# ImpulseAdventure/JPEGsnoop

Measured on AMD Instinct MI355X. Metric: Mpixels/sec decoded (baseline 4:2:0 JPEG) at 1/2/4/8 GPUs; bit-exact vs ref, higher is better.
Workload: dtype u8/i16 entropy+DIB, f32 IDCT+colour; 1 GPU; 1024 x 1920x1080 baseline 4:2:0 q85 JPEG per GPU (64 distinct seeds replicated; BASELINE config 3, config 4 at 8 GPUs), HBM->HBM (T1); images_per_gpu=1024, distinct=64, subsampling=4:2:0, quality=85, parallelism=single, decode_form=two halves on two streams (library default)

## Files before the change

jpegsnoop_amd/csrc/jsnoop_host.cpp:

```cpp
#include <hip/hip_runtime.h>
#include <math.h>
#include <stdarg.h>
#include <stdio.h>
#include <stdlib.h>
#include <string.h>
#include <string>
#include <vector>
#include <chrono>
#include <algorithm>
#include <atomic>
#include "../../include/jsnoop_gpu.h"
#include "jsnoop_types.h"
#include "jsnoop_launch.h"
#include "jsnoop_host.h"
#include "jsnoop_bytes.h"

static thread_local std::string g_err;
void js_set_error(const char* fmt, ...)
{
    char buf[1024]; va_list ap; va_start(ap, fmt); vsnprintf(buf, sizeof buf, fmt, ap); va_end(ap); g_err = buf;
}
#define HIP_TRY(expr) do { hipError_t e_ = (expr); if (e_ != hipSuccess) { \
    js_set_error("%s failed: %s (%s:%d)", #expr, hipGetErrorString(e_), __FILE__, __LINE__); return -1; } } while (0)

// ... 411 lines not shown
        syb[n + 1 + i] = snw; snw += (im.n_subseq + JS_SY_THREADS - JS_SY_HALO - 1) / (JS_SY_THREADS - JS_SY_HALO);
        max_mcu_h = std::max(max_mcu_h, im.mcu_h); max_mcu_w = std::max(max_mcu_w, im.mcu_w);
        wg[i] = wgs; wgs += std::max(1u, (nmcu + 8 * mcus_per_wave - 1) / (8 * mcus_per_wave));
    }
    usb[n] = usc; usb[2 * n + 1] = us4; syb[n] = syw; syb[2 * n + 1] = snw; us_chunks = usc; sy_wgs = syw; sn_wgs = snw; seg_words = segw; mcu_bytes = mcub;
    wg[n] = wgs; total_wgs = wgs; rec_words = recw; total_blocks = blocks; dib_bytes = dibb; side_words = side; total_subseq = subs; ustr_bytes = ustr;
    if (grow(&dev.raw, &cap.raw, raw_bytes + 64) || grow(&dev.coef, &cap.coef, blocks * 128) || grow(&dev.dccum, &cap.dccum, blocks * 2 + 64) ||
        grow(&dev.dib, &cap.dib, dibb) || grow(&dev.side, &cap.side, side * 4) || grow(&dev.imgs, &cap.imgs, n * sizeof(JsImage)) ||
        grow(&dev.tables, &cap.tables, tables.size() * sizeof(JsTableSet)) || grow(&dev.wg_base, &cap.wg_base, (n + 1) * 4) ||
        grow(&dev.sel, &cap.sel, n * 4) || grow(&dev.sums, &cap.sums, n * 8) || grow(&dev.ustr, &cap.ustr, ustr + 64) ||
        grow(&dev.sub, &cap.sub, subs * 24 + 64 + js_sync_list_words(subs, (uint32_t)n) * 4) || grow(&dev.probe, &cap.probe, 1024) || grow(&dev.seg, &cap.seg, segw * 4 + 64) ||
        grow(&dev.chunk_keep, &cap.chunk_keep, (size_t)usc * 4 + 64) || grow(&dev.chunk_rst, &cap.chunk_rst, (size_t)usc * 4 + 64) ||
        grow(&dev.us_base, &cap.us_base, 2 * (n + 1) * 4) || grow(&dev.sy_base, &cap.sy_base, 2 * (n + 1) * 4) ||
        grow(&dev.mcu_rst, &cap.mcu_rst, mcub + 64) || grow(&dev.dc_parts, &cap.dc_parts, JS_DC_PARTS_BYTES) || grow(&dev.ustr_lin, &cap.ustr_lin, ustr + 64) || grow(&dev.flags, &cap.flags, n * 8 + 64) ||
        grow(&dev.us_state, &cap.us_state, (size_t)usc * 8 + 64)) return -1;
    HIP_TRY(hipMemsetAsync(dev.us_state, 0, (size_t)usc * 8 + 64, stream)); us_epoch = 0; us_ticket_base[0] = us_ticket_base[1] = 0;
    if (opt_want_planes && grow(&dev.planes, &cap.planes, plane * 2)) return -1;
    { uint32_t most = 0; for (size_t i = 0; i < n; i++) most = std::max(most, wg[i + 1] - wg[i]); if (most > 64 && grow(&dev.wg_part, &cap.wg_part, (size_t)wgs * 16 + 64)) return -1; }
    cand_blk = max_blk; cand_rounds = (cand_fits && sub_wl == 4) ? cand_want : -1;
    cand_half = cand_rounds >= 0 && tune.write_lanes != 1 && (subs <= 40960 || tune.write_lanes == 2);
    if (cand_rounds >= 0 && (grow(&dev.cand, &cap.cand, js_cand_bytes(subs)) || grow(&dev.cand_req, &cap.cand_req, n * JS_CAND_REQ_WORDS * 4))) return -1;
    event_words = opt_events ? (uint64_t)n * (1 + JS_EV_WORDS * JS_EV_MAX) : 0;
    if (event_words && grow(&dev.events, &cap.events, event_words * 4)) return -1;
    tab_rows = 1; tab_lut2 = 0; uint32_t tdc = 1, tac = 1;
    for (const JsTableSet& t : tables) { tab_rows = std::max(tab_rows, t.n_rows); tab_lut2 = std::max(tab_lut2, t.lut2_used); tdc = std::max(tdc, t.n_dc_rows); tac = std::max(tac, t.n_ac_rows); }
    tab_rows_w = tdc | (tac << 8);
    HIP_TRY(hipMemcpyAsync(dev.raw, pinned, raw_bytes, hipMemcpyHostToDevice, stream));
    {
        const size_t sz[5] = { n * sizeof(JsImage), tables.size() * sizeof(JsTableSet), (n + 1) * 4, 2 * (n + 1) * 4, 2 * (n + 1) * 4 };
        const void* src[5] = { imgs.data(), tables.data(), wg.data(), usb.data(), syb.data() };
        void* dst[5] = { dev.imgs, dev.tables, dev.wg_base, dev.us_base, dev.sy_base };
// ... 73 lines not shown
{
    HIP_TRY(hipSetDevice(device));
    if (!uploaded && upload()) return -1;
    const uint32_t n = (uint32_t)imgs.size();
    last_form = (!force_generic && dc_fast_applies()) ? 2 : 1;
    side_done.assign(n, 0); side_mode.assign(n, 0); side_anoms.assign(n, std::vector<uint32_t>()); side_chunk_ok.assign(n, 0); side_events.assign(n, std::vector<uint32_t>()); side_pre.assign(n, 0); side_requests = 0;
    JsRange r_("jsnoop:decode (enqueue)");
    if (js_prog_count(this)) return decode_progressive(timed);
    if (timed) HIP_TRY(hipEventRecord(ev[0], stream));
    us_epoch = us_epoch % 255u + 1u;
    bool parallel_ok = !opt_force_exact; if (parallel_ok) { parallel_ok = false; for (const JsTableSet& t : tables) parallel_ok = parallel_ok || t.lut_ok; }
    if (!parallel_ok) {
        HIP_TRY(hipMemsetAsync(dev.coef, 0, total_blocks * 128, stream));
        HIP_TRY(hipMemsetAsync(dev.dccum, 0, total_blocks * 2, stream));
    }
    js_launch_clear3(stream, dev.side, side_words * 4, dev.mcu_rst, mcu_bytes, dev.flags, (size_t)n * 8, parallel_ok ? dev.imgs : nullptr, n);
    if (event_words) HIP_TRY(hipMemsetAsync(dev.events, 0, event_words * 4, stream));
    if (timed) HIP_TRY(hipEventRecord(ev[1], stream));
    last_timed_split = false;
    if (split_parts == 2 && parallel_ok && !event_words) {
        if (ensure_aux()) return -1;
        const uint32_t n0 = n / 2; hipStream_t s2 = aux[0];
        HIP_TRY(hipEventRecord(aux_ev[0], stream)); HIP_TRY(hipStreamWaitEvent(s2, aux_ev[0], 0));
        if (js_parallel_entropy_part(this, stream, 0, n0, timed ? ev : nullptr, aux_ev[2], 1) < 0) return -1;
        HIP_TRY(hipStreamWaitEvent(s2, aux_ev[2], 0));
        if (timed) { HIP_TRY(hipEventRecord(ev2[0], s2)); HIP_TRY(hipEventRecord(ev2[1], s2)); }
        if (js_parallel_entropy_part(this, s2, n0, n - n0, timed ? ev2 : nullptr) < 0) return -1;
        last_used_parallel = true;
        if (timed) { HIP_TRY(hipEventRecord(ev[7], stream)); HIP_TRY(hipEventRecord(ev2[7], s2)); }
        { JsRange r2_("jsnoop:idct+colour"); if (launch_back_end_part(stream, 0, n0) || launch_back_end_part(s2, n0, n - n0)) return -1; }
        if (timed) { HIP_TRY(hipEventRecord(ev[8], stream)); HIP_TRY(hipEventRecord(ev2[8], s2)); last_timed_split = true; }
// ... 764 lines not shown
```

jpegsnoop_amd/csrc/jsnoop_host.h:

```cpp
#pragma once
#include <hip/hip_runtime.h>
#include <stdint.h>
#include <string>
#include <utility>
#include <vector>
#include "../../include/jsnoop_gpu.h"
#include "jsnoop_types.h"

struct JsTables {
    uint16_t dqt_nat[4][64], dqt_zz[4][64]; int dqt_sel[256];
    int      dht_sel[2][5];
    uint32_t dht_setmax[2], dht_size[2][4];
    uint32_t dht_bitlen[2][4][JS_DHT_CODES], dht_bits[2][4][JS_DHT_CODES], dht_mask[2][4][JS_DHT_CODES], dht_code[2][4][JS_DHT_CODES];
    uint32_t dht_fast[2][4][2 << JS_FAST_BITS];
    uint32_t dht_histo_unused[1];
    int      details_set; uint32_t dim_x, dim_y, num_sof, num_sos, precision;
    uint32_t samp_h[256], samp_v[256];
    int      rst_en; uint32_t rst_interval;
};

struct JsnoopBatch;
struct JsProgBatch;

struct JsnoopDecoder {
// ... 68 lines not shown
    bool last_timed_split = false;
    bool last_used_parallel = false;
    int  last_form = 0;
    bool force_generic = false;
    bool private_no_log = false;
    bool dc_fast_applies() const;
    int  redecode_generic();
    int  ensure_generic();
    uint32_t* d_side_tmp = nullptr; size_t side_tmp_cap = 0;
    uint8_t* pinned; size_t pinned_cap; uint64_t raw_bytes;
    uint8_t* d2h_land = nullptr;
    uint8_t* h_desc = nullptr; size_t h_desc_cap = 0; hipEvent_t ev_up = nullptr;
    int  d2h_staged(void* dst, const void* src, size_t bytes);
    JsDeviceArenas dev; JsArenaCaps cap;
    bool uploaded;
    uint32_t us_ticket_base[2] = { 0, 0 };
    uint32_t us_epoch = 0;
    uint64_t total_blocks, dib_bytes, side_words, total_subseq, ustr_bytes, seg_words, mcu_bytes; uint32_t total_wgs, strips_per_wg, us_chunks, sy_wgs, sn_wgs, max_mcu_h, max_mcu_w;
    int cand_rounds = -1; uint32_t cand_blk = 0; bool cand_half = false;
    int sync_rounds;
    int sync_launches; int sub_wl;
    uint32_t tab_rows, tab_lut2, tab_rows_w;
    hipEvent_t ev[JSNOOP_NUM_STAGES + 1];
    enum { kAux = 4 };
    hipStream_t aux[kAux] = { nullptr, nullptr, nullptr, nullptr }; hipEvent_t aux_ev[kAux + 1] = { nullptr, nullptr, nullptr, nullptr, nullptr };
    int ensure_aux();
    JsProgBatch* prog = nullptr;
    int  add_progressive(JsnoopDecoder* d, const uint8_t* file, size_t len);
    int  decode_progressive(bool timed);
    int  sync_progressive();
    float lut[64][64]; float* d_lut;
// ... 61 lines not shown
```

jpegsnoop_amd/csrc/jsnoop_kernels.hip:

```cpp
#include <hip/hip_runtime.h>
#include <stdint.h>
#include <atomic>
#include "jsnoop_types.h"
#include "jsnoop_launch.h"

#define WAVE 64
#define WBALLOT(x) __builtin_amdgcn_ballot_w64(static_cast<bool>(x))

__device__ __constant__ uint8_t c_zigzag[64] = {
     0, 1, 8,16, 9, 2, 3,10, 17,24,32,25,18,11, 4, 5,
    12,19,26,33,40,48,41,34, 27,20,13, 6, 7,14,21,28,
    35,42,49,56,57,50,43,36, 29,22,15,23,30,37,44,51,
    58,59,52,45,38,31,39,46, 53,60,61,54,47,55,62,63 };

enum { RSV_OK, RSV_EOB, RSV_UNDERFLOW, RSV_RST_TERM };
enum { SB_OK, SB_BADMARK, SB_RST };

struct ExactReader {
    const uint8_t* file; uint32_t flen;
    const JsTableSet* ts;
    uint32_t* histo;
    uint32_t buff, vacant, ptr, ptr_first;
    uint32_t pos0, pos1, pos2, pos3, err0, err1, err2, err3, latch, num, align;
    uint32_t scan_end, scan_bad, cur_err, restart_read;
// ... 1215 lines not shown
void js_launch_idct_probe(hipStream_t st, const float* lut_t, const int16_t* coef64, float* out64)
{ hipLaunchKernelGGL(k_idct_probe, dim3(1), dim3(64), 64 * 64 * sizeof(float) + LIST_BYTES, st, lut_t, coef64, out64); }
void js_launch_color_probe(hipStream_t st, int y, int cb, int cr, uint32_t* out)
{ hipLaunchKernelGGL(k_color_probe, dim3(1), dim3(1), 0, st, y, cb, cr, out); }
void js_launch_bright_probe(hipStream_t st, const JsImage* imgs, uint32_t img, const uint32_t* side, const int16_t* planes, uint32_t* out8)
{ hipLaunchKernelGGL(k_bright_probe, dim3(1), dim3(1), 0, st, imgs, img, side, planes, out8); }
void js_launch_color_sweep(hipStream_t st, uint32_t* out)
{ hipLaunchKernelGGL(k_color_sweep, dim3(1u << 16), dim3(256), 0, st, out); }
void js_launch_color_stats(hipStream_t st, const JsImage* imgs, uint32_t img, const int16_t* planes, int hist_en, uint32_t* stats)
{ hipLaunchKernelGGL(k_color_stats, dim3(512), dim3(ST_THREADS), 0, st, imgs, img, planes, (uint32_t)(hist_en != 0), stats); }
void js_launch_clip_order(hipStream_t st, const JsImage* imgs, uint32_t img, const int16_t* planes, uint32_t budget, uint32_t* out6)
{ hipLaunchKernelGGL(k_clip_order, dim3(1), dim3(1024), 0, st, imgs, img, planes, budget, out6); }
void js_launch_tiff_pack(hipStream_t st, const JsImage* imgs, uint32_t img, const uint8_t* dib, const int16_t* planes, int mode, uint8_t* out)
{ hipLaunchKernelGGL(k_tiff_pack, dim3(1024), dim3(256), 0, st, imgs, img, dib, planes, mode, out); }
__global__ void __launch_bounds__(256) k_clear3(uint4* __restrict__ a, size_t na, uint4* __restrict__ b, size_t nb, uint4* __restrict__ c, size_t nc,
                                                const JsImage* __restrict__ imgs, uint32_t nimg, uint32_t* __restrict__ side)
{
    const uint4 z = make_uint4(0, 0, 0, 0);
    const size_t ns = imgs ? (size_t)nimg * (JS_SIDE_HISTO / 4) : 0;
    for (size_t i = (size_t)blockIdx.x * 256 + threadIdx.x; i < ns + na + nb + nc; i += (size_t)gridDim.x * 256) {
        if (i < ns) reinterpret_cast<uint4*>(side + imgs[i / (JS_SIDE_HISTO / 4)].side_off)[i % (JS_SIDE_HISTO / 4)] = z;
        else if (i < ns + na) a[i - ns] = z; else if (i < ns + na + nb) b[i - ns - na] = z; else c[i - ns - na - nb] = z;
    }
}
void js_launch_clear3(hipStream_t st, void* a, size_t a_bytes, void* b, size_t b_bytes, void* c, size_t c_bytes, const JsImage* imgs, uint32_t nimg)
{
    const size_t na = imgs ? 0 : (a_bytes + 15) / 16, nb = (b_bytes + 15) / 16, nc = (c_bytes + 15) / 16, tot = na + nb + nc + (imgs ? (size_t)nimg * (JS_SIDE_HISTO / 4) : 0);
    if (!tot) return;
    const uint32_t wgs = (uint32_t)std::min<size_t>(2048, (tot + 1023) / 1024);
    hipLaunchKernelGGL(k_clear3, dim3(wgs), dim3(256), 0, st, (uint4*)a, na, (uint4*)b, nb, (uint4*)c, nc, imgs, nimg, (uint32_t*)a);
}
__global__ void __launch_bounds__(256) k_clear5(uint32_t* __restrict__ a, size_t na, uint32_t* __restrict__ b, size_t nb, uint32_t* __restrict__ c, size_t nc,
                                                uint32_t* __restrict__ d, size_t nd, uint32_t* __restrict__ e, size_t ne)
{
    for (size_t i = (size_t)blockIdx.x * 256 + threadIdx.x; i < na + nb + nc + nd + ne; i += (size_t)gridDim.x * 256) {
        if (i < na) a[i] = 0u; else if (i < na + nb) b[i - na] = 0u; else if (i < na + nb + nc) c[i - na - nb] = 0u;
        else if (i < na + nb + nc + nd) d[i - na - nb - nc] = 0u; else e[i - na - nb - nc - nd] = 0u;
    }
}
void js_launch_clear5(hipStream_t st, uint32_t* a, size_t na, uint32_t* b, size_t nb, uint32_t* c, size_t nc, uint32_t* d, size_t nd, uint32_t* e, size_t ne)
{
    const size_t tot = na + nb + nc + nd + ne;
    if (!tot) return;
    hipLaunchKernelGGL(k_clear5, dim3((uint32_t)std::min<size_t>(1024, (tot + 1023) / 1024)), dim3(256), 0, st, a, na, b, nb, c, nc, d, nd, e, ne);
}
// ... 26 lines not shown
#define F_RST_MISALIGN  0x0008u
#define F_SHORT         0x0010u
#define F_NOSYNC        0x0080u
#define F_BAD_EDGE      0x0100u

template <int WL> __device__ __forceinline__ uint32_t phys_word(uint32_t W) { return WL == 4 ? W : (W & ~((64u << WL) - 1u)) | ((W & ((1u << WL) - 1u)) << 6) | ((W >> WL) & 63u); }
template <int WL> __device__ __forceinline__ uint32_t phys_byte(uint32_t B) { return (phys_word<WL>(B >> 2) << 2) | (B & 3u); }

struct UsBytes { uint32_t keep_mask, rst_mask; };

__device__ __forceinline__ uint32_t us_zero_bytes(uint32_t x)
{
    const uint32_t nz = ((x & 0x7F7F7F7Fu) + 0x7F7F7F7Fu) | x;
    return (((~nz & 0x80808080u) >> 7) * 0x10204080u) >> 28;
}
__device__ __forceinline__ UsBytes us_classify(const uint8_t* __restrict__ raw, uint64_t o16, uint64_t s, uint64_t e, uint4* words = nullptr)
{
    UsBytes r; r.keep_mask = 0; r.rst_mask = 0;
    if (o16 + 16 <= s || o16 >= e) return r;
    const uint4 v = *reinterpret_cast<const uint4*>(raw + o16);
    if (words) *words = v;
    const uint32_t w[4] = { v.x, v.y, v.z, v.w };
    uint32_t prev = o16 > s ? raw[o16 - 1] : 0u;
    const uint32_t next16 = (o16 + 16 < e) ? raw[o16 + 16] : 0u;
    if (o16 > s && o16 + 17 <= e) {
        uint32_t ff = 0, rc = 0, zb = 0;
        #pragma unroll
        for (int q = 0; q < 4; q++) { ff |= us_zero_bytes(~w[q]) << (4 * q); rc |= us_zero_bytes((w[q] & 0xF8F8F8F8u) ^ 0xD0D0D0D0u) << (4 * q); zb |= us_zero_bytes(w[q]) << (4 * q); }
        const uint32_t rc_next = (next16 & 0xF8u) == 0xD0u ? 1u : 0u;
        const uint32_t is_rst = ff & ((rc >> 1) | (rc_next << 15));
        const uint32_t after_ff = ((ff << 1) | (prev == 0xFFu ? 1u : 0u)) & 0xFFFFu & (zb | rc);
        r.keep_mask = ~(after_ff | is_rst) & 0xFFFFu; r.rst_mask = is_rst;
        return r;
    }
    #pragma unroll
    for (int j = 0; j < 16; j++) {
        const uint64_t o = o16 + j;
        const uint32_t b = (w[j >> 2] >> ((j & 3) * 8)) & 255u;
        const uint32_t nb = j < 15 ? ((w[(j + 1) >> 2] >> (((j + 1) & 3) * 8)) & 255u) : next16;
        const bool in = o >= s && o < e;
        const bool is_rst = in && b == 0xFF && (o + 1 < e) && nb >= 0xD0 && nb <= 0xD7;
        const bool drop = (prev == 0xFF && o > s && (b == 0x00 || (b >= 0xD0 && b <= 0xD7))) || is_rst;
        if (in && !drop) r.keep_mask |= 1u << j;
        if (is_rst) r.rst_mask |= 1u << j;
        prev = b;
    }
// ... 158 lines not shown
    const uint32_t* s32 = reinterpret_cast<const uint32_t*>(s_out);
    for (uint32_t w = threadIdx.x; w * 4 < hi_b; w += US_THREADS) {
        if (w * 4 >= lo_b && w * 4 + 4 <= hi_b) reinterpret_cast<uint32_t*>(dst)[w] = phase ? __builtin_amdgcn_alignbyte(s32[w], s32[w - 1], 4u - phase) : s32[w];
        else for (uint32_t b = max(w * 4, lo_b); b < min(w * 4 + 4, hi_b); b++) dst[b] = s_out[b - phase];
    }
}

#define US_SUPER 4
template <int WL>
__global__ void __launch_bounds__(US_THREADS) k_unstuff_fused(const JsImage* __restrict__ imgs, const uint32_t* __restrict__ us_base, const uint32_t* __restrict__ us4_base, uint32_t nimg,
                                                              const uint8_t* __restrict__ raw, uint32_t* __restrict__ chunk_keep, uint32_t* __restrict__ chunk_rst,
                                                              uint8_t* __restrict__ ustr, uint32_t* __restrict__ seg_tab, unsigned long long* __restrict__ us_state, uint32_t epoch,
                                                              uint32_t* __restrict__ side, uint32_t* __restrict__ flags, uint32_t* __restrict__ ticket, uint32_t ticket_base)
{
    constexpr uint32_t PADSH = WL + 2;
    __shared__ __attribute__((aligned(4))) uint8_t s_out[US_SUPER * US_CHUNK + ((US_SUPER * US_CHUNK) >> WL) + 16];
    __shared__ uint32_t wk[US_SUPER][US_THREADS / 64], wr[US_SUPER][US_THREADS / 64];
    __shared__ uint32_t s_excl[2];
    __shared__ uint32_t s_bid;
    if (threadIdx.x == 0) s_bid = atomicAdd(ticket, 1u) - ticket_base;
    __syncthreads();
    const uint32_t sw = s_bid + us4_base[0];
    const uint32_t img = find_image(us4_base, nimg, sw);
    const JsImage& im = imgs[img];
    const uint32_t sc = sw - us4_base[img], nsc = us4_base[img + 1] - us4_base[img];
    const uint32_t c0 = sc * US_SUPER, nc = us_base[img + 1] - us_base[img], wgc = us_base[img] + c0;
    const uint64_t s = im.file_off + im.scan_start, e = s + im.scan_len;
    const uint32_t lane = threadIdx.x & 63, wave = threadIdx.x >> 6;
    UsBytes c[US_SUPER]; uint4 v[US_SUPER]; uint32_t pk[US_SUPER], pr[US_SUPER];
    #pragma unroll
    for (uint32_t q = 0; q < US_SUPER; q++) {
        v[q] = make_uint4(0u, 0u, 0u, 0u); c[q].keep_mask = 0; c[q].rst_mask = 0;
        if (c0 + q < nc) c[q] = us_classify(raw, (s & ~15ull) + (uint64_t)(c0 + q) * US_CHUNK + threadIdx.x * 16, s, e, &v[q]);
    }
    #pragma unroll
    for (uint32_t q = 0; q < US_SUPER; q++) {
        uint32_t x = __popc(c[q].keep_mask) | (__popc(c[q].rst_mask) << 16);
        for (int off = 1; off < 64; off <<= 1) { const uint32_t a = __shfl_up(x, off); if (lane >= (uint32_t)off) x += a; }
        pk[q] = x & 0xFFFFu; pr[q] = x >> 16;
        if (lane == 63) { wk[q][wave] = pk[q]; wr[q][wave] = pr[q]; }
    }
    __syncthreads();
    uint32_t agg_k = 0, agg_r = 0, lk[US_SUPER], lr[US_SUPER], ck[US_SUPER], cr[US_SUPER];
    #pragma unroll
    for (uint32_t q = 0; q < US_SUPER; q++) {
        ck[q] = agg_k; cr[q] = agg_r;
        lk[q] = agg_k + pk[q] - __popc(c[q].keep_mask); lr[q] = agg_r + pr[q] - __popc(c[q].rst_mask);
        #pragma unroll
        for (uint32_t w = 0; w < US_THREADS / 64; w++) { if (w < wave) { lk[q] += wk[q][w]; lr[q] += wr[q][w]; } agg_k += wk[q][w]; agg_r = us_sat_add(agg_r, wr[q][w]); }
    }
    if (sc && threadIdx.x == 0) __hip_atomic_store(&us_state[sw], us_pack(epoch, US_ST_AGG, agg_k, agg_r), __ATOMIC_RELAXED, __HIP_MEMORY_SCOPE_AGENT);
    #pragma unroll
    for (uint32_t q = 0; q < US_SUPER; q++) if (c[q].keep_mask) {
        const uint32_t w4[4] = { v[q].x, v[q].y, v[q].z, v[q].w };
        uint32_t g = lk[q];
        #pragma unroll
        for (int j = 0; j < 16; j++) if (c[q].keep_mask & (1u << j)) { s_out[g + ((g >> PADSH) << 2)] = (uint8_t)(w4[j >> 2] >> ((j & 3) * 8)); g++; }
    }
    if (wave == 0) {
        uint32_t ek, er;
        us_lookback(us_state, sw, sc, epoch, lane, ek, er);
        if (lane == 0) {
            __hip_atomic_store(&us_state[sw], us_pack(epoch, US_ST_INC, ek + agg_k, us_sat_add(er, agg_r)), __ATOMIC_RELAXED, __HIP_MEMORY_SCOPE_AGENT);
            s_excl[0] = ek; s_excl[1] = er;
            if (sc + 1 == nsc) {
                const uint32_t run_k = ek + agg_k, run_r = us_sat_add(er, agg_r);
                uint32_t* sd = side + im.side_off; uint32_t* st = seg_tab + im.seg_off;
                sd[10] = run_k; sd[11] = run_r + 1;
                st[0] = 0;
                if (run_r + 2 <= im.seg_cap) st[run_r + 1] = run_k; else { FLAG_OR(flags, img, F_OVERRUN); ANOM_MIN(flags, img, ANOM_KEY(0u, AK_MIRROR)); }
            }
        }
// ... 1462 lines not shown
    const uint32_t m0 = part * per, m1 = min(nmcu, m0 + per);
    DcSeg* sm = summaries + (size_t)img * DC_PARTS_MAX;
    if (m0 >= nmcu) { if (!apply && threadIdx.x == 0) { const DcSeg z = { 0, 0, 0, 0 }; sm[part] = z; } return; }
    __shared__ DcSeg s_w[DC_THREADS / 64];
    int16_t* d = dccum + im.coef_off; const uint8_t* rf = mcu_rst + im.mcu_off;
    DcSeg carry = { 0, 0, 0, 0 };
    if (apply) { for (uint32_t q = 0; q < part; q++) carry = dc_combine(carry, sm[q]); carry.r = 0; }
    const bool small = im.blk_per_mcu <= 6;
    if (!apply) { if (small) dc_scan_range<6, false>(im, d, rf, s_w, m0, m1, carry, sm + part); else dc_scan_range<JS_MAX_BLK_PER_MCU, false>(im, d, rf, s_w, m0, m1, carry, sm + part); }
    else        { if (small) dc_scan_range<6, true>(im, d, rf, s_w, m0, m1, carry, nullptr);  else dc_scan_range<JS_MAX_BLK_PER_MCU, true>(im, d, rf, s_w, m0, m1, carry, nullptr); }
}

void js_launch_unstuff(hipStream_t st, int wl, const JsImage* imgs, const uint32_t* us_base, uint32_t nimg, uint32_t total_chunks, const uint8_t* raw,
                       uint32_t* chunk_keep, uint32_t* chunk_rst, uint8_t* ustr_lin, uint8_t* ustr, uint32_t* seg_tab, uint32_t* side, uint32_t* flags,
                       const uint32_t* sy_base, uint32_t sy_wgs, unsigned long long* us_state, uint32_t epoch, const uint32_t* us4_base, uint32_t total_super,
                       uint32_t* ticket, uint32_t* ticket_base )
{
    if (!total_chunks) return;
    if (us_state && wl != 4 && us4_base) {
#define JS_USF(W) hipLaunchKernelGGL(k_unstuff_fused<W>, dim3(total_super), dim3(US_THREADS), 0, st, imgs, us_base, us4_base, nimg, raw, chunk_keep, chunk_rst, ustr, seg_tab, us_state, epoch, side, flags, ticket, *ticket_base)
        if (wl == 5) JS_USF(5); else if (wl == 6) JS_USF(6); else if (wl == 7) JS_USF(7); else JS_USF(8);
#undef JS_USF
        *ticket_base += total_super;
        return;
    }
    if (us_state) {
        hipLaunchKernelGGL(k_unstuff_write<true>, dim3(total_chunks), dim3(US_THREADS), 0, st, imgs, us_base, nimg, raw, chunk_keep, chunk_rst, wl == 4 ? ustr : ustr_lin, seg_tab, 0u,
                           (uint32_t*)nullptr, us_state, epoch, side, flags, ticket, *ticket_base);
        *ticket_base += total_chunks;
    } else {
        hipLaunchKernelGGL(k_unstuff_count, dim3(total_chunks), dim3(US_THREADS), 0, st, imgs, us_base, nimg, raw, chunk_keep, chunk_rst);
        hipLaunchKernelGGL(k_unstuff_scan, dim3(nimg), dim3(256), 0, st, imgs, us_base, chunk_keep, chunk_rst, seg_tab, side, flags);
        hipLaunchKernelGGL(k_unstuff_write<false>, dim3(total_chunks), dim3(US_THREADS), 0, st, imgs, us_base, nimg, raw, chunk_keep, chunk_rst, wl == 4 ? ustr : ustr_lin, seg_tab, 0u,
                           (uint32_t*)nullptr, (unsigned long long*)nullptr, 0u, (uint32_t*)nullptr, (uint32_t*)nullptr, (uint32_t*)nullptr, 0u);
    }
    if (wl == 4) return;
    if (wl == 6) hipLaunchKernelGGL(k_interleave<6>, dim3(sy_wgs * 4), dim3(256), 0, st, imgs, sy_base, nimg, side, ustr_lin, ustr);
    else if (wl == 8) hipLaunchKernelGGL(k_interleave<8>, dim3(sy_wgs * 4), dim3(256), 0, st, imgs, sy_base, nimg, side, ustr_lin, ustr);
    else if (wl == 7) hipLaunchKernelGGL(k_interleave<7>, dim3(sy_wgs * 4), dim3(256), 0, st, imgs, sy_base, nimg, side, ustr_lin, ustr);
    else hipLaunchKernelGGL(k_interleave<5>, dim3(sy_wgs * 4), dim3(256), 0, st, imgs, sy_base, nimg, side, ustr_lin, ustr);
}
static SubArrays sub_arrays(uint32_t* sub, uint64_t n) { SubArrays a; a.out_p = sub; a.out_s = sub + n; a.in_p = sub + 2 * n; a.in_s = sub + 3 * n; a.nblk = sub + 4 * n; a.base = sub + 5 * n; return a; }
static size_t subtabs_bytes_host(uint32_t tab_rows, uint32_t tab_lut2, bool pairs = false)
{ return pairs ? (size_t)tab_rows * (4u << JS_L1_BITS) + (size_t)tab_lut2 * 4 : (size_t)tab_rows * (2u << JS_L1_BITS) + (((size_t)tab_lut2 * 2 + 15) & ~15ull) + 3 * 64 * 4; }
// ... 545 lines not shown
```

jpegsnoop_amd/csrc/jsnoop_launch.h:

```cpp
#pragma once
#include <hip/hip_runtime.h>
#include <stdint.h>
#include "jsnoop_types.h"

void js_launch_entropy_exact(hipStream_t st, const JsImage* imgs, const uint32_t* sel, uint32_t nsel, const JsTableSet* tables,
                             const uint8_t* raw, int16_t* coef, int16_t* dccum, uint32_t* side, int side_only, uint32_t* events);
int  js_launch_idct_color(hipStream_t st, const JsImage* imgs, const uint32_t* wg_base, uint32_t nimg, uint32_t total_wgs, uint32_t tile_bytes,
                          const float* lut_t, const int16_t* coef, const int16_t* dccum, uint8_t* dib, int16_t* planes, uint32_t* side,
                          int layout ,
                          unsigned long long* wg_part );
void js_launch_unaligned_probe(hipStream_t st, void* buf48);
void js_launch_idct_probe(hipStream_t st, const float* lut_t, const int16_t* coef64, float* out64);
void js_launch_clear3(hipStream_t st, void* a, size_t a_bytes, void* b, size_t b_bytes, void* c, size_t c_bytes, const JsImage* imgs = nullptr, uint32_t nimg = 0);
void js_launch_clear5(hipStream_t st, uint32_t* a, size_t na, uint32_t* b, size_t nb, uint32_t* c, size_t nc, uint32_t* d, size_t nd, uint32_t* e, size_t ne);
void js_launch_dib_checksum(hipStream_t st, const JsImage* imgs, uint32_t nimg, const uint8_t* dib, unsigned long long* sums);
void js_launch_color_probe(hipStream_t st, int y, int cb, int cr, uint32_t* out);
void js_launch_bright_probe(hipStream_t st, const JsImage* imgs, uint32_t img, const uint32_t* side, const int16_t* planes , uint32_t* out8);
#define JS_STATS_WORDS 2482
#define JS_STATS_DEV_WORDS 2496
void js_launch_color_stats(hipStream_t st, const JsImage* imgs, uint32_t img, const int16_t* planes, int hist_en, uint32_t* stats);
void js_launch_clip_order(hipStream_t st, const JsImage* imgs, uint32_t img, const int16_t* planes, uint32_t budget, uint32_t* out6);
void js_launch_tiff_pack(hipStream_t st, const JsImage* imgs, uint32_t img, const uint8_t* dib, const int16_t* planes, int mode, uint8_t* out);
void js_launch_color_sweep(hipStream_t st, uint32_t* out );
void js_launch_unstuff(hipStream_t st, int wl, const JsImage* imgs, const uint32_t* us_base, uint32_t nimg, uint32_t total_chunks, const uint8_t* raw,
                       uint32_t* chunk_keep, uint32_t* chunk_rst, uint8_t* ustr_lin, uint8_t* ustr, uint32_t* seg_tab, uint32_t* side, uint32_t* flags,
                       const uint32_t* sy_base, uint32_t sy_wgs, unsigned long long* us_state , uint32_t epoch,
                       const uint32_t* us4_base , uint32_t total_super,
                       uint32_t* ticket , uint32_t* ticket_base );
void js_launch_sync(hipStream_t st, int wl, uint32_t tab_rows, uint32_t tab_lut2, const JsImage* imgs, const uint32_t* sy_base, uint32_t nimg, uint32_t total_wgs, const JsTableSet* tables,
                    const uint8_t* ustr, const uint32_t* seg_tab, const uint32_t* side, uint32_t* sub, uint64_t nsub, int first_pass, uint32_t it_max = 0 );
#define JS_SYR_SLOTS 12
#define JS_SYR_ROUNDS 8
size_t js_sync_list_words(uint64_t nsub, uint32_t nimg);
void js_launch_sync_rounds(hipStream_t st, int wl, uint32_t tab_rows, uint32_t tab_lut2, const JsImage* imgs, const uint32_t* sn_base, uint32_t sn_wgs, const uint32_t* sy_base, uint32_t sy_wgs,
                           uint32_t nimg, const JsTableSet* tables, const uint8_t* ustr, const uint32_t* seg_tab, const uint32_t* side, uint32_t* sub, uint64_t nsub,
                           uint32_t* lists , uint32_t* rcnt , int rounds);
#define JS_SY_THREADS 256
#define JS_SY_HALO    2
#define JS_CAND_MAX_BLK 6
#define JS_CAND_REQ_WORDS 12
size_t js_cand_bytes(uint64_t nsub);
void js_launch_cand_sync(hipStream_t st, int wl, uint32_t tab_rows, uint32_t tab_lut2, const JsImage* imgs, const uint32_t* sy_base, uint32_t nimg, uint32_t sy_wgs, uint32_t max_blk,
                         const JsTableSet* tables, const uint8_t* ustr, const uint32_t* seg_tab, const uint32_t* side, uint32_t* sub, uint64_t nsub, uint32_t* cand, uint32_t* req, int fill_rounds,
// ... 35 lines not shown
```

jpegsnoop_amd/csrc/jsnoop_parallel.cpp:

```cpp
#include <stdio.h>
#include <stdlib.h>
#include <string.h>
#include <vector>
#include <algorithm>
#include "jsnoop_host.h"
#include "jsnoop_launch.h"

#define HIP_TRY(expr) do { hipError_t e_ = (expr); if (e_ != hipSuccess) { \
    js_set_error("%s failed: %s (%s:%d)", #expr, hipGetErrorString(e_), __FILE__, __LINE__); return -1; } } while (0)

void js_build_parallel_luts(JsTableSet* ts, uint32_t ncomp)
{
    ts->lut_ok = 0; ts->n_rows = 0; ts->lut2_used = 0;
    memset(ts->lut1, 0, sizeof ts->lut1); memset(ts->lut2, 0, sizeof ts->lut2); memset(ts->slot_row, 0, sizeof ts->slot_row); memset(ts->lutp, 0, sizeof ts->lutp); memset(ts->lut2p, 0, sizeof ts->lut2p);
    uint32_t l2_used = 0;
    for (uint32_t slot = 0; slot < ncomp * 2; slot++) {
        const uint32_t n = ts->size[slot]; const bool is_dc = (slot & 1) == 0;
        if (n == 0 || n > 256) return;
        uint32_t prev_len = 0; uint64_t next_code = 0;
        for (uint32_t i = 0; i < n; i++) {
            const uint32_t len = ts->bitlen[slot][i], bits = ts->bits[slot][i], sym = ts->code[slot][i];
            if (len < 1 || len > 16 || len < prev_len || sym > 255) return;
            if (ts->mask[slot][i] != (0xFFFFFFFFu << (32 - len))) return;
            next_code <<= (len - prev_len);
// ... 232 lines not shown
}

int js_parallel_entropy_part(JsnoopBatch* b, hipStream_t st, uint32_t i0, uint32_t n, hipEvent_t* evs, hipEvent_t after_stage, int which_stage)
{
    const uint32_t N = (uint32_t)b->imgs.size();
    uint32_t* sub = (uint32_t*)b->dev.sub;
    const JsImage* imgs = b->dev.imgs + i0;
    const uint32_t* us_base = b->dev.us_base + i0; const uint32_t* sy_base = b->dev.sy_base + i0; const uint32_t* sn_base = b->dev.sy_base + (N + 1) + i0;
    uint32_t* flags = b->dev.flags + 2 * (size_t)i0;
    const uint32_t us_chunks = b->h_us_base[i0 + n] - b->h_us_base[i0], sy_wgs = b->h_sy_base[i0 + n] - b->h_sy_base[i0], sn_wgs = b->h_sn_base[i0 + n] - b->h_sn_base[i0];
    roctxRangePushA("jsnoop:unstuff");
    js_launch_unstuff(st, b->sub_wl, imgs, us_base, n, us_chunks, b->dev.raw, b->dev.chunk_keep, b->dev.chunk_rst,
                      b->dev.ustr_lin, b->dev.ustr, b->dev.seg, b->dev.side, flags, sy_base, sy_wgs,
                      (b->tune.cross_checks & JSNOOP_XC_UNSTUFF_3PASS) ? nullptr : b->dev.us_state, b->us_epoch,
                      b->dev.us_base + (N + 1) + i0, b->h_us4_base[i0 + n] - b->h_us4_base[i0],
                      reinterpret_cast<uint32_t*>(b->dev.us_state + b->us_chunks) + (i0 ? 1 : 0), &b->us_ticket_base[i0 ? 1 : 0]);
    roctxRangePop();
    if (evs) HIP_TRY(hipEventRecord(evs[2], st));
    if (after_stage && which_stage == 1) HIP_TRY(hipEventRecord(after_stage, st));
    roctxRangePushA("jsnoop:sub-sequence sync");
    if (b->cand_rounds >= 0) {
        js_launch_cand_sync(st, b->sub_wl, b->tab_rows, b->tab_lut2, imgs, sy_base, n, sy_wgs, b->cand_blk, b->dev.tables, b->dev.ustr, b->dev.seg, b->dev.side, sub, b->total_subseq,
                            b->dev.cand, b->dev.cand_req + (size_t)i0 * JS_CAND_REQ_WORDS, b->cand_rounds, b->cand_half ? 1 : 0);
        if (b->tune.debug & JSNOOP_DBG_CAND_LINKS) js_debug_cand_links(b, st, i0, n);
        if (b->tune.cross_checks & JSNOOP_XC_CAND_VERIFY) {
            js_launch_sync(st, b->sub_wl, b->tab_rows, b->tab_lut2, imgs, sn_base, n, sn_wgs, b->dev.tables, b->dev.ustr, b->dev.seg, b->dev.side, sub, b->total_subseq, 2);
            js_launch_sync(st, b->sub_wl, b->tab_rows, b->tab_lut2, imgs, sn_base, n, sn_wgs, b->dev.tables, b->dev.ustr, b->dev.seg, b->dev.side, sub, b->total_subseq, 0);
        }
    } else if (b->sync_rounds > 0) {
        uint32_t* lists = sub + 6 * (size_t)b->total_subseq + 16;
        js_launch_sync_rounds(st, b->sub_wl, b->tab_rows, b->tab_lut2, imgs, sn_base, sn_wgs, sy_base, sy_wgs, n, b->dev.tables, b->dev.ustr, b->dev.seg, b->dev.side, sub, b->total_subseq,
// ... 519 lines not shown
```

Baseline: 176,700 Mpixels/s.

## Reset unstuff tickets on device and vectorize byte-unstuff classify and compaction

The dynamic-ticket counters for the unstuff kernels are now zeroed by the clear kernel on each decode, so the host no longer tracks a running ticket base. The fused unstuff kernel switches to a classify path that only inspects bytes following 0xFF, using dot-product packing and byte permutes. It also compacts kept bytes in registers with shift-and-mask steps and writes them to zero-initialised shared memory through atomic ORs, replacing per-byte stores. The cost is an extra shared-memory clear and atomics per thread, plus wave-divergent loops when a chunk has many stuffed bytes.

```diff
diff --git a/jpegsnoop_amd/csrc/jsnoop_host.cpp b/jpegsnoop_amd/csrc/jsnoop_host.cpp
--- a/jpegsnoop_amd/csrc/jsnoop_host.cpp
+++ b/jpegsnoop_amd/csrc/jsnoop_host.cpp
@@ -449,7 +449,7 @@
         grow(&dev.us_base, &cap.us_base, 2 * (n + 1) * 4) || grow(&dev.sy_base, &cap.sy_base, 2 * (n + 1) * 4) ||
         grow(&dev.mcu_rst, &cap.mcu_rst, mcub + 64) || grow(&dev.dc_parts, &cap.dc_parts, JS_DC_PARTS_BYTES) || grow(&dev.ustr_lin, &cap.ustr_lin, ustr + 64) || grow(&dev.flags, &cap.flags, n * 8 + 64) ||
         grow(&dev.us_state, &cap.us_state, (size_t)usc * 8 + 64)) return -1;
-    HIP_TRY(hipMemsetAsync(dev.us_state, 0, (size_t)usc * 8 + 64, stream)); us_epoch = 0; us_ticket_base[0] = us_ticket_base[1] = 0;
+    HIP_TRY(hipMemsetAsync(dev.us_state, 0, (size_t)usc * 8 + 64, stream)); us_epoch = 0;
     if (opt_want_planes && grow(&dev.planes, &cap.planes, plane * 2)) return -1;
     { uint32_t most = 0; for (size_t i = 0; i < n; i++) most = std::max(most, wg[i + 1] - wg[i]); if (most > 64 && grow(&dev.wg_part, &cap.wg_part, (size_t)wgs * 16 + 64)) return -1; }
     cand_blk = max_blk; cand_rounds = (cand_fits && sub_wl == 4) ? cand_want : -1;
@@ -553,7 +553,7 @@
         HIP_TRY(hipMemsetAsync(dev.coef, 0, total_blocks * 128, stream));
         HIP_TRY(hipMemsetAsync(dev.dccum, 0, total_blocks * 2, stream));
     }
-    js_launch_clear3(stream, dev.side, side_words * 4, dev.mcu_rst, mcu_bytes, dev.flags, (size_t)n * 8, parallel_ok ? dev.imgs : nullptr, n);
+    js_launch_clear3(stream, dev.side, side_words * 4, dev.mcu_rst, mcu_bytes, dev.flags, (size_t)n * 8, parallel_ok ? dev.imgs : nullptr, n, reinterpret_cast<uint32_t*>(dev.us_state + us_chunks));
     if (event_words) HIP_TRY(hipMemsetAsync(dev.events, 0, event_words * 4, stream));
     if (timed) HIP_TRY(hipEventRecord(ev[1], stream));
     last_timed_split = false;
diff --git a/jpegsnoop_amd/csrc/jsnoop_host.h b/jpegsnoop_amd/csrc/jsnoop_host.h
--- a/jpegsnoop_amd/csrc/jsnoop_host.h
+++ b/jpegsnoop_amd/csrc/jsnoop_host.h
@@ -106,7 +106,6 @@
     int  d2h_staged(void* dst, const void* src, size_t bytes);
     JsDeviceArenas dev; JsArenaCaps cap;
     bool uploaded;
-    uint32_t us_ticket_base[2] = { 0, 0 };
     uint32_t us_epoch = 0;
     uint64_t total_blocks, dib_bytes, side_words, total_subseq, ustr_bytes, seg_words, mcu_bytes; uint32_t total_wgs, strips_per_wg, us_chunks, sy_wgs, sn_wgs, max_mcu_h, max_mcu_w;
     int cand_rounds = -1; uint32_t cand_blk = 0; bool cand_half = false;
diff --git a/jpegsnoop_amd/csrc/jsnoop_kernels.hip b/jpegsnoop_amd/csrc/jsnoop_kernels.hip
--- a/jpegsnoop_amd/csrc/jsnoop_kernels.hip
+++ b/jpegsnoop_amd/csrc/jsnoop_kernels.hip
@@ -1253,21 +1253,22 @@
 void js_launch_tiff_pack(hipStream_t st, const JsImage* imgs, uint32_t img, const uint8_t* dib, const int16_t* planes, int mode, uint8_t* out)
 { hipLaunchKernelGGL(k_tiff_pack, dim3(1024), dim3(256), 0, st, imgs, img, dib, planes, mode, out); }
 __global__ void __launch_bounds__(256) k_clear3(uint4* __restrict__ a, size_t na, uint4* __restrict__ b, size_t nb, uint4* __restrict__ c, size_t nc,
-                                                const JsImage* __restrict__ imgs, uint32_t nimg, uint32_t* __restrict__ side)
+                                                const JsImage* __restrict__ imgs, uint32_t nimg, uint32_t* __restrict__ side, uint32_t* __restrict__ tickets)
 {
     const uint4 z = make_uint4(0, 0, 0, 0);
+    if (tickets && blockIdx.x == 0 && threadIdx.x < 2) tickets[threadIdx.x] = 0u;
     const size_t ns = imgs ? (size_t)nimg * (JS_SIDE_HISTO / 4) : 0;
     for (size_t i = (size_t)blockIdx.x * 256 + threadIdx.x; i < ns + na + nb + nc; i += (size_t)gridDim.x * 256) {
         if (i < ns) reinterpret_cast<uint4*>(side + imgs[i / (JS_SIDE_HISTO / 4)].side_off)[i % (JS_SIDE_HISTO / 4)] = z;
         else if (i < ns + na) a[i - ns] = z; else if (i < ns + na + nb) b[i - ns - na] = z; else c[i - ns - na - nb] = z;
     }
 }
-void js_launch_clear3(hipStream_t st, void* a, size_t a_bytes, void* b, size_t b_bytes, void* c, size_t c_bytes, const JsImage* imgs, uint32_t nimg)
+void js_launch_clear3(hipStream_t st, void* a, size_t a_bytes, void* b, size_t b_bytes, void* c, size_t c_bytes, const JsImage* imgs, uint32_t nimg, uint32_t* tickets)
 {
     const size_t na = imgs ? 0 : (a_bytes + 15) / 16, nb = (b_bytes + 15) / 16, nc = (c_bytes + 15) / 16, tot = na + nb + nc + (imgs ? (size_t)nimg * (JS_SIDE_HISTO / 4) : 0);
     if (!tot) return;
     const uint32_t wgs = (uint32_t)std::min<size_t>(2048, (tot + 1023) / 1024);
-    hipLaunchKernelGGL(k_clear3, dim3(wgs), dim3(256), 0, st, (uint4*)a, na, (uint4*)b, nb, (uint4*)c, nc, imgs, nimg, (uint32_t*)a);
+    hipLaunchKernelGGL(k_clear3, dim3(wgs), dim3(256), 0, st, (uint4*)a, na, (uint4*)b, nb, (uint4*)c, nc, imgs, nimg, (uint32_t*)a, tickets);
 }
 __global__ void __launch_bounds__(256) k_clear5(uint32_t* __restrict__ a, size_t na, uint32_t* __restrict__ b, size_t nb, uint32_t* __restrict__ c, size_t nc,
                                                 uint32_t* __restrict__ d, size_t nd, uint32_t* __restrict__ e, size_t ne)
@@ -1324,6 +1325,7 @@
     const uint32_t nz = ((x & 0x7F7F7F7Fu) + 0x7F7F7F7Fu) | x;
     return (((~nz & 0x80808080u) >> 7) * 0x10204080u) >> 28;
 }
+template <bool BEHIND_FF = false>
 __device__ __forceinline__ UsBytes us_classify(const uint8_t* __restrict__ raw, uint64_t o16, uint64_t s, uint64_t e, uint4* words = nullptr)
 {
     UsBytes r; r.keep_mask = 0; r.rst_mask = 0;
@@ -1334,12 +1336,33 @@
     uint32_t prev = o16 > s ? raw[o16 - 1] : 0u;
     const uint32_t next16 = (o16 + 16 < e) ? raw[o16 + 16] : 0u;
     if (o16 > s && o16 + 17 <= e) {
-        uint32_t ff = 0, rc = 0, zb = 0;
+        if (!BEHIND_FF) {
+            uint32_t ff = 0, rc = 0, zb = 0;
+            #pragma unroll
+            for (int q = 0; q < 4; q++) { ff |= us_zero_bytes(~w[q]) << (4 * q); rc |= us_zero_bytes((w[q] & 0xF8F8F8F8u) ^ 0xD0D0D0D0u) << (4 * q); zb |= us_zero_bytes(w[q]) << (4 * q); }
+            const uint32_t rc_next = (next16 & 0xF8u) == 0xD0u ? 1u : 0u;
+            const uint32_t is_rst = ff & ((rc >> 1) | (rc_next << 15));
+            const uint32_t after_ff = ((ff << 1) | (prev == 0xFFu ? 1u : 0u)) & 0xFFFFu & (zb | rc);
+            r.keep_mask = ~(after_ff | is_rst) & 0xFFFFu; r.rst_mask = is_rst;
+            return r;
+        }
+        uint32_t f[4];
         #pragma unroll
-        for (int q = 0; q < 4; q++) { ff |= us_zero_bytes(~w[q]) << (4 * q); rc |= us_zero_bytes((w[q] & 0xF8F8F8F8u) ^ 0xD0D0D0D0u) << (4 * q); zb |= us_zero_bytes(w[q]) << (4 * q); }
-        const uint32_t rc_next = (next16 & 0xF8u) == 0xD0u ? 1u : 0u;
-        const uint32_t is_rst = ff & ((rc >> 1) | (rc_next << 15));
-        const uint32_t after_ff = ((ff << 1) | (prev == 0xFFu ? 1u : 0u)) & 0xFFFFu & (zb | rc);
+        for (int q = 0; q < 4; q++) f[q] = ((w[q] & 0x7F7F7F7Fu) + 0x01010101u) & w[q] & 0x80808080u;
+        const uint32_t ff = (__builtin_amdgcn_udot4(f[1], 0x80402010u, __builtin_amdgcn_udot4(f[0], 0x08040201u, 0u, false), false) >> 7) |
+                            (__builtin_amdgcn_udot4(f[3], 0x80402010u, __builtin_amdgcn_udot4(f[2], 0x08040201u, 0u, false), false) << 1);
+        uint32_t behind = (ff << 1) | (prev == 0xFFu ? 1u : 0u), after_ff = 0, code = 0;
+        while (WBALLOT(behind)) {
+            if (behind) {
+                const uint32_t j = __builtin_ctz(behind), sel = (j & 7u) | 0x0C0C0C00u;
+                behind &= behind - 1u;
+                const uint32_t lo = __builtin_amdgcn_perm(w[1], w[0], sel), hi = __builtin_amdgcn_perm(w[3], w[2], sel);
+                const uint32_t b = j >= 16u ? next16 : j >= 8u ? hi : lo;
+                const uint32_t is_code = (b & 0xF8u) == 0xD0u ? 1u : 0u;
+                after_ff |= (b == 0u ? 1u : is_code) << j; code |= is_code << j;
+            }
+        }
+        const uint32_t is_rst = (code >> 1) & 0xFFFFu;
         r.keep_mask = ~(after_ff | is_rst) & 0xFFFFu; r.rst_mask = is_rst;
         return r;
     }
@@ -1528,11 +1551,20 @@
                                                               uint32_t* __restrict__ side, uint32_t* __restrict__ flags, uint32_t* __restrict__ ticket, uint32_t ticket_base)
 {
     constexpr uint32_t PADSH = WL + 2;
-    __shared__ __attribute__((aligned(4))) uint8_t s_out[US_SUPER * US_CHUNK + ((US_SUPER * US_CHUNK) >> WL) + 16];
+    constexpr uint32_t OUT16 = (US_SUPER * US_CHUNK + ((US_SUPER * US_CHUNK) >> WL) + 16 + 15) / 16;
+    __shared__ __attribute__((aligned(16))) uint8_t s_out[OUT16 * 16];
+    __shared__ uint4 s_low[17];
     __shared__ uint32_t wk[US_SUPER][US_THREADS / 64], wr[US_SUPER][US_THREADS / 64];
     __shared__ uint32_t s_excl[2];
     __shared__ uint32_t s_bid;
     if (threadIdx.x == 0) s_bid = atomicAdd(ticket, 1u) - ticket_base;
+    for (uint32_t i = threadIdx.x; i < OUT16; i += US_THREADS) reinterpret_cast<uint4*>(s_out)[i] = make_uint4(0u, 0u, 0u, 0u);
+    if (threadIdx.x < 17) {
+        uint32_t m[4];
+        #pragma unroll
+        for (int k = 0; k < 4; k++) { const int b = (int)threadIdx.x - 4 * k; m[k] = b <= 0 ? 0u : b >= 4 ? 0xFFFFFFFFu : (1u << (8 * b)) - 1u; }
+        s_low[threadIdx.x] = make_uint4(m[0], m[1], m[2], m[3]);
+    }
     __syncthreads();
     const uint32_t sw = s_bid + us4_base[0];
     const uint32_t img = find_image(us4_base, nimg, sw);
@@ -1545,7 +1577,7 @@
     #pragma unroll
     for (uint32_t q = 0; q < US_SUPER; q++) {
         v[q] = make_uint4(0u, 0u, 0u, 0u); c[q].keep_mask = 0; c[q].rst_mask = 0;
-        if (c0 + q < nc) c[q] = us_classify(raw, (s & ~15ull) + (uint64_t)(c0 + q) * US_CHUNK + threadIdx.x * 16, s, e, &v[q]);
+        if (c0 + q < nc) c[q] = us_classify<true>(raw, (s & ~15ull) + (uint64_t)(c0 + q) * US_CHUNK + threadIdx.x * 16, s, e, &v[q]);
     }
     #pragma unroll
     for (uint32_t q = 0; q < US_SUPER; q++) {
@@ -1565,11 +1597,38 @@
     }
     if (sc && threadIdx.x == 0) __hip_atomic_store(&us_state[sw], us_pack(epoch, US_ST_AGG, agg_k, agg_r), __ATOMIC_RELAXED, __HIP_MEMORY_SCOPE_AGENT);
     #pragma unroll
-    for (uint32_t q = 0; q < US_SUPER; q++) if (c[q].keep_mask) {
-        const uint32_t w4[4] = { v[q].x, v[q].y, v[q].z, v[q].w };
-        uint32_t g = lk[q];
-        #pragma unroll
-        for (int j = 0; j < 16; j++) if (c[q].keep_mask & (1u << j)) { s_out[g + ((g >> PADSH) << 2)] = (uint8_t)(w4[j >> 2] >> ((j & 3) * 8)); g++; }
+    for (uint32_t q = 0; q < US_SUPER; q++) {
+        const uint32_t km = c[q].keep_mask;
+        const uint32_t holes = __popc(~km & ((1u << (32 - __clz(km))) - 1u));
+        if (WBALLOT(holes > 3u)) {
+            if (km) {
+                const uint32_t w4[4] = { v[q].x, v[q].y, v[q].z, v[q].w };
+                uint32_t g = lk[q];
+                #pragma unroll
+                for (int j = 0; j < 16; j++) if (km & (1u << j)) { s_out[g + ((g >> PADSH) << 2)] = (uint8_t)(w4[j >> 2] >> ((j & 3) * 8)); g++; }
+            }
+            continue;
+        }
+        uint32_t w0 = v[q].x, w1 = v[q].y, w2 = v[q].z, w3 = v[q].w, k2 = km;
+        while (WBALLOT(k2 & (k2 + 1u))) {
+            const uint32_t p = __builtin_ctz(~k2);
+            const uint4 m = s_low[p];
+            const uint32_t s0 = __builtin_amdgcn_alignbyte(w1, w0, 1u), s1 = __builtin_amdgcn_alignbyte(w2, w1, 1u), s2 = __builtin_amdgcn_alignbyte(w3, w2, 1u), s3 = w3 >> 8;
+            w0 = (w0 & m.x) | (s0 & ~m.x); w1 = (w1 & m.y) | (s1 & ~m.y); w2 = (w2 & m.z) | (s2 & ~m.z); w3 = (w3 & m.w) | (s3 & ~m.w);
+            const uint32_t below = (1u << p) - 1u;
+            k2 = (k2 & below) | ((k2 >> 1) & ~below);
+        }
+        if (km) {
+            const uint4 m = s_low[__popc(km)];
+            w0 &= m.x; w1 &= m.y; w2 &= m.z; w3 &= m.w;
+            const uint32_t g = lk[q], t = (0u - g) & 3u, wi = (g + 3u) >> 2;
+            uint32_t* s32w = reinterpret_cast<uint32_t*>(s_out);
+            if (t) __hip_atomic_fetch_or(&s32w[(wi - 1u) + ((wi - 1u) >> WL)], __builtin_amdgcn_alignbyte(w0, 0u, t), __ATOMIC_RELAXED, __HIP_MEMORY_SCOPE_WORKGROUP);
+            __hip_atomic_fetch_or(&s32w[wi + (wi >> WL)], __builtin_amdgcn_alignbyte(w1, w0, t), __ATOMIC_RELAXED, __HIP_MEMORY_SCOPE_WORKGROUP);
+            __hip_atomic_fetch_or(&s32w[(wi + 1u) + ((wi + 1u) >> WL)], __builtin_amdgcn_alignbyte(w2, w1, t), __ATOMIC_RELAXED, __HIP_MEMORY_SCOPE_WORKGROUP);
+            __hip_atomic_fetch_or(&s32w[(wi + 2u) + ((wi + 2u) >> WL)], __builtin_amdgcn_alignbyte(w3, w2, t), __ATOMIC_RELAXED, __HIP_MEMORY_SCOPE_WORKGROUP);
+            __hip_atomic_fetch_or(&s32w[(wi + 3u) + ((wi + 3u) >> WL)], __builtin_amdgcn_alignbyte(0u, w3, t), __ATOMIC_RELAXED, __HIP_MEMORY_SCOPE_WORKGROUP);
+        }
     }
     if (wave == 0) {
         uint32_t ek, er;
@@ -3062,20 +3121,18 @@
 void js_launch_unstuff(hipStream_t st, int wl, const JsImage* imgs, const uint32_t* us_base, uint32_t nimg, uint32_t total_chunks, const uint8_t* raw,
                        uint32_t* chunk_keep, uint32_t* chunk_rst, uint8_t* ustr_lin, uint8_t* ustr, uint32_t* seg_tab, uint32_t* side, uint32_t* flags,
                        const uint32_t* sy_base, uint32_t sy_wgs, unsigned long long* us_state, uint32_t epoch, const uint32_t* us4_base, uint32_t total_super,
-                       uint32_t* ticket, uint32_t* ticket_base )
+                       uint32_t* ticket )
 {
     if (!total_chunks) return;
     if (us_state && wl != 4 && us4_base) {
-#define JS_USF(W) hipLaunchKernelGGL(k_unstuff_fused<W>, dim3(total_super), dim3(US_THREADS), 0, st, imgs, us_base, us4_base, nimg, raw, chunk_keep, chunk_rst, ustr, seg_tab, us_state, epoch, side, flags, ticket, *ticket_base)
+#define JS_USF(W) hipLaunchKernelGGL(k_unstuff_fused<W>, dim3(total_super), dim3(US_THREADS), 0, st, imgs, us_base, us4_base, nimg, raw, chunk_keep, chunk_rst, ustr, seg_tab, us_state, epoch, side, flags, ticket, 0u)
         if (wl == 5) JS_USF(5); else if (wl == 6) JS_USF(6); else if (wl == 7) JS_USF(7); else JS_USF(8);
 #undef JS_USF
-        *ticket_base += total_super;
         return;
     }
     if (us_state) {
         hipLaunchKernelGGL(k_unstuff_write<true>, dim3(total_chunks), dim3(US_THREADS), 0, st, imgs, us_base, nimg, raw, chunk_keep, chunk_rst, wl == 4 ? ustr : ustr_lin, seg_tab, 0u,
-                           (uint32_t*)nullptr, us_state, epoch, side, flags, ticket, *ticket_base);
-        *ticket_base += total_chunks;
+                           (uint32_t*)nullptr, us_state, epoch, side, flags, ticket, 0u);
     } else {
         hipLaunchKernelGGL(k_unstuff_count, dim3(total_chunks), dim3(US_THREADS), 0, st, imgs, us_base, nimg, raw, chunk_keep, chunk_rst);
         hipLaunchKernelGGL(k_unstuff_scan, dim3(nimg), dim3(256), 0, st, imgs, us_base, chunk_keep, chunk_rst, seg_tab, side, flags);
diff --git a/jpegsnoop_amd/csrc/jsnoop_launch.h b/jpegsnoop_amd/csrc/jsnoop_launch.h
--- a/jpegsnoop_amd/csrc/jsnoop_launch.h
+++ b/jpegsnoop_amd/csrc/jsnoop_launch.h
@@ -11,7 +11,7 @@
                           unsigned long long* wg_part );
 void js_launch_unaligned_probe(hipStream_t st, void* buf48);
 void js_launch_idct_probe(hipStream_t st, const float* lut_t, const int16_t* coef64, float* out64);
-void js_launch_clear3(hipStream_t st, void* a, size_t a_bytes, void* b, size_t b_bytes, void* c, size_t c_bytes, const JsImage* imgs = nullptr, uint32_t nimg = 0);
+void js_launch_clear3(hipStream_t st, void* a, size_t a_bytes, void* b, size_t b_bytes, void* c, size_t c_bytes, const JsImage* imgs = nullptr, uint32_t nimg = 0, uint32_t* tickets = nullptr);
 void js_launch_clear5(hipStream_t st, uint32_t* a, size_t na, uint32_t* b, size_t nb, uint32_t* c, size_t nc, uint32_t* d, size_t nd, uint32_t* e, size_t ne);
 void js_launch_dib_checksum(hipStream_t st, const JsImage* imgs, uint32_t nimg, const uint8_t* dib, unsigned long long* sums);
 void js_launch_color_probe(hipStream_t st, int y, int cb, int cr, uint32_t* out);
@@ -26,7 +26,7 @@
                        uint32_t* chunk_keep, uint32_t* chunk_rst, uint8_t* ustr_lin, uint8_t* ustr, uint32_t* seg_tab, uint32_t* side, uint32_t* flags,
                        const uint32_t* sy_base, uint32_t sy_wgs, unsigned long long* us_state , uint32_t epoch,
                        const uint32_t* us4_base , uint32_t total_super,
-                       uint32_t* ticket , uint32_t* ticket_base );
+                       uint32_t* ticket );
 void js_launch_sync(hipStream_t st, int wl, uint32_t tab_rows, uint32_t tab_lut2, const JsImage* imgs, const uint32_t* sy_base, uint32_t nimg, uint32_t total_wgs, const JsTableSet* tables,
                     const uint8_t* ustr, const uint32_t* seg_tab, const uint32_t* side, uint32_t* sub, uint64_t nsub, int first_pass, uint32_t it_max = 0 );
 #define JS_SYR_SLOTS 12
diff --git a/jpegsnoop_amd/csrc/jsnoop_parallel.cpp b/jpegsnoop_amd/csrc/jsnoop_parallel.cpp
--- a/jpegsnoop_amd/csrc/jsnoop_parallel.cpp
+++ b/jpegsnoop_amd/csrc/jsnoop_parallel.cpp
@@ -270,7 +270,7 @@
                       b->dev.ustr_lin, b->dev.ustr, b->dev.seg, b->dev.side, flags, sy_base, sy_wgs,
                       (b->tune.cross_checks & JSNOOP_XC_UNSTUFF_3PASS) ? nullptr : b->dev.us_state, b->us_epoch,
                       b->dev.us_base + (N + 1) + i0, b->h_us4_base[i0 + n] - b->h_us4_base[i0],
-                      reinterpret_cast<uint32_t*>(b->dev.us_state + b->us_chunks) + (i0 ? 1 : 0), &b->us_ticket_base[i0 ? 1 : 0]);
+                      reinterpret_cast<uint32_t*>(b->dev.us_state + b->us_chunks) + (i0 ? 1 : 0));
     roctxRangePop();
     if (evs) HIP_TRY(hipEventRecord(evs[2], st));
     if (after_stage && which_stage == 1) HIP_TRY(hipEventRecord(after_stage, st));
```

After: 174,100 Mpixels/s. 0.985x the previous value.
